# jie0530/act-plus-plus

Hardware: AMD Instinct MI355X
Metric: policy steps/sec (4x480x640 cams, chunk=100, bs=8) (higher is better)
Workload: dtype f32 (f16x3 split products: 3 fp16 MFMAs per fp32 product, fp32 accumulate); 1 GPU; ACT eval policy query: 4 cams 480x640 u8, chunk 100, hidden 512, ff 3200, 4 enc + 7 dec layers (layer 0 live), per-GPU batch 8, + temporal ensemble; per_gpu_batch=8, global_batch=8, parallelism=replicas x1

## Files before the change

act-plus-plus_amd/csrc/attn.hip:

```cpp
#include "common.h"
#include "dropout.h"
#include "split16.h"
#include <cstdio>
#include <cstdlib>

namespace {

constexpr bool ATTN_NOPF = true;
constexpr int KT = 64;
typedef _Float16 h16x8 __attribute__((ext_vector_type(8)));

__device__ __forceinline__ void attn_block_coords(int& bx, int& by, int& bz) {
    const int gx = gridDim.x, gy = gridDim.y;
    const int total = gx * gy * (int)gridDim.z;
    const int lin = ((int)blockIdx.z * gy + (int)blockIdx.y) * gx + (int)blockIdx.x;
    const int xcd = lin & 7, q = total >> 3, r = total & 7;
    const int base = (xcd < r) ? xcd * (q + 1) : r * (q + 1) + (xcd - r) * q;
    const int flat = base + (lin >> 3);
    bx = flat % gx;
    const int rest = flat / gx;
    by = rest % gy;
    bz = rest / gy;
}

template <int HD>
__global__ __launch_bounds__(256) void attn_f32_kernel(AttnArgs p, int nsplit, int chunk) {
    constexpr int HH = HD / 2;
    constexpr int DT = (HD + 31) / 32;
    constexpr int VD = DT * 32;
    constexpr int KS = HD + 4;
    __shared__ __attribute__((aligned(16))) float s_k[KT * KS];
    __shared__ __attribute__((aligned(16))) float s_v[KT * VD];

    const int t = threadIdx.x, lane = t & 63, wave = t >> 6;
    const int li = lane & 31, lh = lane >> 5;
    int bx, h, b;
    attn_block_coords(bx, h, b);
    const int split = bx % nsplit;
    const int q = (bx / nsplit) * 128 + wave * 32 + li;
    const int k_begin = split * chunk;
    const int k_end = (k_begin + chunk < p.Nk) ? k_begin + chunk : p.Nk;
    const bool qok = q < p.Nq;

    const float qscale = p.scale * 1.4426950408889634f;
    const float* Qp = p.Q + (int64_t)b * p.q_bs + (int64_t)(qok ? q : 0) * p.q_rs + h * HD + lh * HH;
    float qreg[HH];
#pragma unroll
    for (int s = 0; s < HH; s += 4) {
        f32x4 v = *reinterpret_cast<const f32x4*>(Qp + s);
#pragma unroll
        for (int j = 0; j < 4; ++j) qreg[s + j] = qok ? v[j] * qscale : 0.f;
    }
    const float* Kb = p.K + (int64_t)b * p.k_bs + h * HD;
    const float* Vb = p.V + (int64_t)b * p.v_bs + h * HD;
    const uint8_t* kpm = p.kpm ? p.kpm + (int64_t)b * p.kpm_bs : nullptr;

    f32x16 O[DT];
#pragma unroll
    for (int d = 0; d < DT; ++d)
#pragma unroll
        for (int e = 0; e < 16; ++e) O[d][e] = 0.f;
// ... 100 lines not shown
                for (int e = 0; e < 16; ++e) {
                    const int kl = sub * 32 + (e & 3) + 8 * (e >> 2) + 4 * lh;
#pragma unroll
                    for (int d = 0; d < DT; ++d) {
                        const float vv = s_v[kl * VD + d * 32 + li];
                        O[d] = __builtin_amdgcn_mfma_f32_32x32x2f32(vv, S[e], O[d], 0, 0, 0);
                    }
                }
            }
        }
        __syncthreads();
    }
    if (qok) {
        if (nsplit == 1) {
            const float inv = 1.f / l_run;
            float* Op = p.O + (int64_t)b * p.o_bs + (int64_t)q * p.o_rs + h * HD;
#pragma unroll
            for (int d = 0; d < DT; ++d)
#pragma unroll
                for (int g = 0; g < 4; ++g) {
                    const int d0 = d * 32 + 8 * g + 4 * lh;
                    if (d0 < HD) {
                        f32x4 o = {O[d][4 * g] * inv, O[d][4 * g + 1] * inv, O[d][4 * g + 2] * inv, O[d][4 * g + 3] * inv};
                        *reinterpret_cast<f32x4*>(Op + d0) = o;
                    }
                }
            if (p.lse && lh == 0) p.lse[((int64_t)b * p.H + h) * p.Nq + q] = m_run * 0.6931471805599453f + logf(l_run);
        } else {
            const int64_t row = (((int64_t)split * p.B + b) * p.H + h) * p.Nq + q;
            float* Op = p.ws + row * HD;
            float* ml = p.ws + (int64_t)nsplit * p.B * p.H * p.Nq * HD + row * 2;
#pragma unroll
            for (int d = 0; d < DT; ++d)
#pragma unroll
                for (int g = 0; g < 4; ++g) {
                    const int d0 = d * 32 + 8 * g + 4 * lh;
                    if (d0 < HD) {
                        f32x4 o = {O[d][4 * g], O[d][4 * g + 1], O[d][4 * g + 2], O[d][4 * g + 3]};
                        *reinterpret_cast<f32x4*>(Op + d0) = o;
                    }
                }
            if (lh == 0) { ml[0] = m_run; ml[1] = l_run; }
        }
    }
}

template <int HD>
__global__ __launch_bounds__(256, 3) void attn_f16x3_kernel(AttnArgs p, int nsplit, int chunk) {
    constexpr int NS = HD / 16;
    constexpr int DT = (HD + 31) / 32;
    constexpr int VD = DT * 32;
    constexpr int KROW = 4 * HD + 16;
    constexpr int VROW = 4 * KT + 16;
    __shared__ __attribute__((aligned(16))) unsigned char s_k[KT * KROW];
    __shared__ __attribute__((aligned(16))) unsigned char s_vt[VD * VROW];
    __shared__ uint8_t s_dead[KT];

    const int t = threadIdx.x, lane = t & 63, wave = t >> 6;
    const int li = lane & 31, lh = lane >> 5;
    int bx, h, b;
    attn_block_coords(bx, h, b);
    const int split = bx % nsplit;
    const int q = (bx / nsplit) * 128 + wave * 32 + li;
    const int k_begin = split * chunk;
    const int k_end = (k_begin + chunk < p.Nk) ? k_begin + chunk : p.Nk;
    const bool qok = q < p.Nq;

    const float qscale = p.scale * 1.4426950408889634f;
    const float* Qp = p.Q + (int64_t)b * p.q_bs + (int64_t)(qok ? q : 0) * p.q_rs + h * HD + lh * 8;
    h16x8 qh[NS], ql[NS];
#pragma unroll
    for (int s = 0; s < NS; ++s) {
        f32x4 v0 = *reinterpret_cast<const f32x4*>(Qp + s * 16);
        f32x4 v1 = *reinterpret_cast<const f32x4*>(Qp + s * 16 + 4);
        const float sc = qok ? qscale : 0.f;
        v0 *= sc; v1 *= sc;
        uint2 h0, l0, h1, l1;
        split16(v0, h0, l0);
        split16(v1, h1, l1);
        qh[s] = __builtin_bit_cast(h16x8, uint4{h0.x, h0.y, h1.x, h1.y});
        ql[s] = __builtin_bit_cast(h16x8, uint4{l0.x, l0.y, l1.x, l1.y});
    }
    const float* Kb = p.K + (int64_t)b * p.k_bs + h * HD;
    const float* Vb = p.V + (int64_t)b * p.v_bs + h * HD;
    const uint8_t* kpm = p.kpm ? p.kpm + (int64_t)b * p.kpm_bs : nullptr;

    f32x16 O[DT];
#pragma unroll
    for (int d = 0; d < DT; ++d)
#pragma unroll
        for (int e = 0; e < 16; ++e) O[d][e] = 0.f;
    float m_run = -INFINITY, l_run = 0.f;

    if (HD < VD) {
        for (int e = t; e < VD * VROW / 4; e += 256) reinterpret_cast<uint32_t*>(s_vt)[e] = 0u;
        __syncthreads();
    }

    constexpr int C4 = HD / 4;
    constexpr int NLK = (KT * C4 + 255) / 256;
    constexpr int NLV = (KT / 2 * C4 + 255) / 256;
    f32x4 pk[NLK], pv[NLV][2];
    auto vc = [&](int e) { return ((e >> 5) % (C4 / 4)) * 4 + (e & 3); };
    auto vkp = [&](int e) { return ((e >> 5) / (C4 / 4)) * 8 + ((e >> 2) & 7); };
    auto fetch = [&](int kt0) {
        const f32x4 z = {0.f, 0.f, 0.f, 0.f};
#pragma unroll
        for (int i = 0; i < NLK; ++i) {
            const int e = t + 256 * i;
            const int kr = e / C4, c = e - kr * C4;
            const int key = kt0 + kr;
            const bool ok = e < KT * C4 && key < k_end;
            const f32x4 kv = *reinterpret_cast<const f32x4*>(Kb + (ok ? (int64_t)key * p.k_rs + c * 4 : 0));
            pk[i] = ok ? kv : z;
        }
#pragma unroll
        for (int i = 0; i < NLV; ++i) {
            const int e = t + 256 * i;
            const int kp = vkp(e), c = vc(e);
#pragma unroll
            for (int u = 0; u < 2; ++u) {
                const int key = kt0 + 2 * kp + u;
                const bool ok = e < KT / 2 * C4 && key < k_end;
                const f32x4 vv = *reinterpret_cast<const f32x4*>(Vb + (ok ? (int64_t)key * p.v_rs + c * 4 : 0));
                pv[i][u] = ok ? vv : z;
            }
        }
    };
    if (!ATTN_NOPF) fetch(k_begin);
    for (int kt0 = k_begin; kt0 < k_end; kt0 += KT) {
        if (ATTN_NOPF) fetch(kt0);
#pragma unroll
        for (int i = 0; i < NLK; ++i) {
            const int e = t + 256 * i;
            if (e < KT * C4) {
                const int kr = e / C4, c = e - kr * C4;
                uint2 hi, lo;
                split16(pk[i], hi, lo);
                *reinterpret_cast<uint2*>(s_k + kr * KROW + c * 8) = hi;
                *reinterpret_cast<uint2*>(s_k + kr * KROW + 2 * HD + c * 8) = lo;
            }
        }
#pragma unroll
        for (int i = 0; i < NLV; ++i) {
            const int e = t + 256 * i;
            if (e < KT / 2 * C4) {
                const int kp = vkp(e), c = vc(e);
                uint2 ha, la, hb, lb;
                split16(pv[i][0], ha, la);
                split16(pv[i][1], hb, lb);
                const int kl = 2 * kp, r = kl & 15;
                const int pos = (kl & ~15) | (r & 3) | ((r & 8) >> 1) | ((r & 4) << 1);
                unsigned char* dst = s_vt + (c * 4) * VROW + pos * 2;
                *reinterpret_cast<uint32_t*>(dst + 0 * VROW) = (ha.x & 0xffffu) | (hb.x << 16);
                *reinterpret_cast<uint32_t*>(dst + 1 * VROW) = (ha.x >> 16) | (hb.x & 0xffff0000u);
                *reinterpret_cast<uint32_t*>(dst + 2 * VROW) = (ha.y & 0xffffu) | (hb.y << 16);
                *reinterpret_cast<uint32_t*>(dst + 3 * VROW) = (ha.y >> 16) | (hb.y & 0xffff0000u);
                *reinterpret_cast<uint32_t*>(dst + 0 * VROW + 2 * KT) = (la.x & 0xffffu) | (lb.x << 16);
                *reinterpret_cast<uint32_t*>(dst + 1 * VROW + 2 * KT) = (la.x >> 16) | (lb.x & 0xffff0000u);
                *reinterpret_cast<uint32_t*>(dst + 2 * VROW + 2 * KT) = (la.y & 0xffffu) | (lb.y << 16);
                *reinterpret_cast<uint32_t*>(dst + 3 * VROW + 2 * KT) = (la.y >> 16) | (lb.y & 0xffff0000u);
            }
        }
        const bool ragged = kt0 + KT > k_end || kpm != nullptr;
        if (ragged && t < KT) {
            const int key = kt0 + t;
            s_dead[t] = (key >= k_end) || (kpm && kpm[key] != 0);
        }
        __syncthreads();
        if (!ATTN_NOPF && kt0 + KT < k_end) fetch(kt0 + KT);
#pragma unroll
        for (int sub = 0; sub < KT / 32; ++sub) {
            const int kb = kt0 + sub * 32;
            if (kb < k_end) {
                f32x16 S;
#pragma unroll
                for (int e = 0; e < 16; ++e) S[e] = 0.f;
                const unsigned char* krow = s_k + (sub * 32 + li) * KROW + lh * 16;
#pragma unroll
                for (int s = 0; s < NS; ++s) {
                    const h16x8 kh = __builtin_bit_cast(h16x8, *reinterpret_cast<const f32x4*>(krow + s * 32));
                    const h16x8 kl = __builtin_bit_cast(h16x8, *reinterpret_cast<const f32x4*>(krow + 2 * HD + s * 32));
                    S = __builtin_amdgcn_mfma_f32_32x32x16_f16(kl, qh[s], S, 0, 0, 0);
                    S = __builtin_amdgcn_mfma_f32_32x32x16_f16(kh, ql[s], S, 0, 0, 0);
                    S = __builtin_amdgcn_mfma_f32_32x32x16_f16(kh, qh[s], S, 0, 0, 0);
                }
                if (ragged) {
#pragma unroll
                    for (int e = 0; e < 16; ++e)
                        if (s_dead[sub * 32 + (e & 3) + 8 * (e >> 2) + 4 * lh]) S[e] = -INFINITY;
                }
                if (p.causal) {
#pragma unroll
                    for (int e = 0; e < 16; ++e)
                        if (kb + (e & 3) + 8 * (e >> 2) + 4 * lh > q) S[e] = -INFINITY;
                }
                float mt = S[0];
#pragma unroll
                for (int e = 1; e < 16; ++e) mt = fmaxf(mt, S[e]);
                mt = fmaxf(mt, __shfl_xor(mt, 32, 64));
                const float m_new = fmaxf(m_run, mt);
                const float m_safe = (m_new == -INFINITY) ? 0.f : m_new;
                const float alpha = __builtin_amdgcn_exp2f(m_run - m_safe);
                float rs = 0.f;
#pragma unroll
                for (int e = 0; e < 16; ++e) {
                    S[e] = __builtin_amdgcn_exp2f(S[e] - m_safe);
                    rs += S[e];
                }
                rs += __shfl_xor(rs, 32, 64);
                l_run = l_run * alpha + rs;
                m_run = m_new;
                if (p.drop_p > 0.f) {
                    const float ds = 1.f / (1.f - p.drop_p);
                    const uint64_t rowbase = (((uint64_t)b * p.H + h) * p.Nq + (qok ? q : 0)) * (uint64_t)p.Nk;
#pragma unroll
                    for (int e = 0; e < 16; ++e) {
                        const int key = kb + (e & 3) + 8 * (e >> 2) + 4 * lh;
                        S[e] = actmi_keep(p.drop_seed, rowbase + key, p.drop_p) ? S[e] * ds : 0.f;
                    }
                }
                h16x8 ph[2], pl[2];
#pragma unroll
                for (int g2 = 0; g2 < 2; ++g2) {
                    const f32x4 a0 = {S[8 * g2], S[8 * g2 + 1], S[8 * g2 + 2], S[8 * g2 + 3]};
                    const f32x4 a1 = {S[8 * g2 + 4], S[8 * g2 + 5], S[8 * g2 + 6], S[8 * g2 + 7]};
                    uint2 h0, l0, h1, l1;
                    split16(a0, h0, l0);
                    split16(a1, h1, l1);
                    ph[g2] = __builtin_bit_cast(h16x8, uint4{h0.x, h0.y, h1.x, h1.y});
                    pl[g2] = __builtin_bit_cast(h16x8, uint4{l0.x, l0.y, l1.x, l1.y});
                }
#pragma unroll
                for (int d = 0; d < DT; ++d) {
#pragma unroll
                    for (int e = 0; e < 16; ++e) O[d][e] *= alpha;
                    const unsigned char* vrow = s_vt + (d * 32 + li) * VROW + sub * 64 + lh * 16;
#pragma unroll
                    for (int g2 = 0; g2 < 2; ++g2) {
                        const h16x8 vh = __builtin_bit_cast(h16x8, *reinterpret_cast<const f32x4*>(vrow + g2 * 32));
                        const h16x8 vl = __builtin_bit_cast(h16x8, *reinterpret_cast<const f32x4*>(vrow + 2 * KT + g2 * 32));
                        O[d] = __builtin_amdgcn_mfma_f32_32x32x16_f16(vl, ph[g2], O[d], 0, 0, 0);
                        O[d] = __builtin_amdgcn_mfma_f32_32x32x16_f16(vh, pl[g2], O[d], 0, 0, 0);
                        O[d] = __builtin_amdgcn_mfma_f32_32x32x16_f16(vh, ph[g2], O[d], 0, 0, 0);
                    }
                }
            }
        }
        __syncthreads();
    }
    if (qok) {
        if (nsplit == 1) {
            const float inv = 1.f / l_run;
            float* Op = p.O + (int64_t)b * p.o_bs + (int64_t)q * p.o_rs + h * HD;
#pragma unroll
            for (int d = 0; d < DT; ++d)
#pragma unroll
                for (int g = 0; g < 4; ++g) {
                    const int d0 = d * 32 + 8 * g + 4 * lh;
                    if (d0 < HD) {
                        f32x4 o = {O[d][4 * g] * inv, O[d][4 * g + 1] * inv, O[d][4 * g + 2] * inv, O[d][4 * g + 3] * inv};
                        *reinterpret_cast<f32x4*>(Op + d0) = o;
                    }
                }
            if (p.lse && lh == 0) p.lse[((int64_t)b * p.H + h) * p.Nq + q] = m_run * 0.6931471805599453f + logf(l_run);
        } else {
            const int64_t row = (((int64_t)split * p.B + b) * p.H + h) * p.Nq + q;
            float* Op = p.ws + row * HD;
            float* ml = p.ws + (int64_t)nsplit * p.B * p.H * p.Nq * HD + row * 2;
#pragma unroll
            for (int d = 0; d < DT; ++d)
#pragma unroll
                for (int g = 0; g < 4; ++g) {
                    const int d0 = d * 32 + 8 * g + 4 * lh;
                    if (d0 < HD) {
                        f32x4 o = {O[d][4 * g], O[d][4 * g + 1], O[d][4 * g + 2], O[d][4 * g + 3]};
                        *reinterpret_cast<f32x4*>(Op + d0) = o;
                    }
                }
            if (lh == 0) { ml[0] = m_run; ml[1] = l_run; }
        }
    }
}


__global__ void attn_combine_kernel(AttnArgs p, int nsplit, int HD) {
    const int64_t idx = (int64_t)blockIdx.x * blockDim.x + threadIdx.x;
    const int D4 = HD / 4;
    const int64_t total = (int64_t)p.B * p.H * p.Nq * D4;
    if (idx >= total) return;
    const int d4 = (int)(idx % D4);
    const int64_t bhq = idx / D4;
    const int q = (int)(bhq % p.Nq);
    const int h = (int)((bhq / p.Nq) % p.H);
    const int b = (int)(bhq / ((int64_t)p.Nq * p.H));
    const int64_t per = (int64_t)p.B * p.H * p.Nq;
    const float* mlb = p.ws + (int64_t)nsplit * per * HD;
    float m = -INFINITY;
    for (int s = 0; s < nsplit; ++s) m = fmaxf(m, mlb[(s * per + bhq) * 2]);
// ... 73 lines not shown
```

act-plus-plus_amd/csrc/conv3.hip:

```cpp
#include "common.h"
#include "split16.h"

namespace {

typedef _Float16 h16x8 __attribute__((ext_vector_type(8)));

constexpr int TR = 4, TW = 32, CH = 64;
constexpr int NTHR = TR * 64;
constexpr int PR = TR + 2, PW = TW + 2;
constexpr int PIX = 272;
constexpr int PATCH = PR * PW * PIX;
constexpr int WROW = 272;
constexpr int WBUF = CH * WROW;
constexpr int SMEM = PATCH + WBUF;

__global__ __launch_bounds__(NTHR) void conv3x3_c64_f16x3_kernel(Conv3Args p, int tiles_w, int tiles_h) {
    extern __shared__ __attribute__((aligned(16))) unsigned char smem[];
    unsigned char* s_patch = smem;
    unsigned char* s_w = smem + PATCH;
    const int t = threadIdx.x, lane = t & 63, wave = t >> 6;
    const int li = lane & 31, lh = lane >> 5;

    int tile;
    {
        const int total = (int)gridDim.x, lin = (int)blockIdx.x;
        const int xcd = lin & 7, q = total >> 3, r = total & 7;
        const int base = (xcd < r) ? xcd * (q + 1) : r * (q + 1) + (xcd - r) * q;
        tile = base + (lin >> 3);
    }
    const int tw = tile % tiles_w; tile /= tiles_w;
    const int th = tile % tiles_h; tile /= tiles_h;
    const int64_t img = tile;
    const int g = (int)(img / p.B);
    const int h0 = th * TR, w0 = tw * TW;
    const float* xin = p.x + img * (int64_t)p.H * p.W * CH;
    const float* wsplit = p.w16 + (int64_t)g * CH * 9 * CH;

    constexpr int WD = 4;
    constexpr int NWG = 1024 / NTHR;
    uint4 wreg[WD][NWG];
    auto fetch_w = [&](int tap, uint4 (&wr)[NWG]) {
#pragma unroll
        for (int i = 0; i < NWG; ++i) {
            const int e = t + NTHR * i;
            const int n = e >> 4, grp = e & 15;
            wr[i] = *reinterpret_cast<const uint4*>(wsplit + ((int64_t)n * 9 + tap) * CH + grp * 4);
        }
    };
    auto commit_w = [&](int buf, const uint4 (&wr)[NWG]) {
        unsigned char* dst = s_w;
#pragma unroll
        for (int i = 0; i < NWG; ++i) {
            const int e = t + NTHR * i;
            const int n = e >> 4, grp = e & 15;
            *reinterpret_cast<uint2*>(dst + n * WROW + grp * 8) = uint2{wr[i].x, wr[i].y};
            *reinterpret_cast<uint2*>(dst + n * WROW + 128 + grp * 8) = uint2{wr[i].z, wr[i].w};
        }
    };
#pragma unroll
    for (int k = 0; k < WD; ++k) fetch_w(k, wreg[k]);

    constexpr int NP = (PR * PW * 16 + NTHR - 1) / NTHR;
    const float xs = p.x_scale_dev ? *p.x_scale_dev : 1.f;
    const unsigned amax_seen = p.amax_out ? __hip_atomic_load(p.amax_out, __ATOMIC_RELAXED, __HIP_MEMORY_SCOPE_AGENT) : 0u;
    f32x4 pv[NP];
#pragma unroll
    for (int i = 0; i < NP; ++i) {
        const int e = t + NTHR * i;
        const int grp = e & 15, pix = e >> 4;
        const int pr = pix / PW, pc = pix - pr * PW;
        const int hi = h0 - 1 + pr, wi = w0 - 1 + pc;
        const bool ok = e < PR * PW * 16 && (unsigned)hi < (unsigned)p.H && (unsigned)wi < (unsigned)p.W;
        const f32x4 v = *reinterpret_cast<const f32x4*>(xin + (ok ? ((int64_t)hi * p.W + wi) * CH + grp * 4 : 0));
        pv[i] = ok ? v : f32x4{0.f, 0.f, 0.f, 0.f};
    }
#pragma unroll
    for (int i = 0; i < NP; ++i) {
        const int e = t + NTHR * i;
        if (e < PR * PW * 16) {
            const int grp = e & 15, pix = e >> 4;
            uint2 hv, lv;
            split16(pv[i] * xs, hv, lv);
            *reinterpret_cast<uint2*>(s_patch + pix * PIX + grp * 8) = hv;
            *reinterpret_cast<uint2*>(s_patch + pix * PIX + 128 + grp * 8) = lv;
        }
    }
    commit_w(0, wreg[0]);
    __syncthreads();

    f32x16 acc[2];
#pragma unroll
    for (int nt = 0; nt < 2; ++nt)
#pragma unroll
        for (int e = 0; e < 16; ++e) acc[nt][e] = 0.f;

#pragma unroll
    for (int tap = 0; tap < 9; ++tap) {
        const int buf = 0;
        if (tap + WD < 9) fetch_w(tap + WD, wreg[tap % WD]);
        const int r = tap / 3, s = tap - r * 3;
        const unsigned char* ap = s_patch + ((wave + r) * PW + li + s) * PIX + lh * 16;
        const unsigned char* bp = s_w + li * WROW + lh * 16;
        uint4 fa[4][2], fb[4][2][2];
#pragma unroll
        for (int ks = 0; ks < 4; ++ks) {
            fa[ks][0] = *reinterpret_cast<const uint4*>(ap + ks * 32);
            fa[ks][1] = *reinterpret_cast<const uint4*>(ap + 128 + ks * 32);
#pragma unroll
            for (int nt = 0; nt < 2; ++nt) {
                fb[ks][nt][0] = *reinterpret_cast<const uint4*>(bp + nt * 32 * WROW + ks * 32);
                fb[ks][nt][1] = *reinterpret_cast<const uint4*>(bp + nt * 32 * WROW + 128 + ks * 32);
            }
        }
#pragma unroll
        for (int ks = 0; ks < 4; ++ks) {
            const h16x8 xh = __builtin_bit_cast(h16x8, fa[ks][0]), xl = __builtin_bit_cast(h16x8, fa[ks][1]);
#pragma unroll
            for (int nt = 0; nt < 2; ++nt) {
                const h16x8 yh = __builtin_bit_cast(h16x8, fb[ks][nt][0]), yl = __builtin_bit_cast(h16x8, fb[ks][nt][1]);
                acc[nt] = __builtin_amdgcn_mfma_f32_32x32x16_f16(xl, yh, acc[nt], 0, 0, 0);
                acc[nt] = __builtin_amdgcn_mfma_f32_32x32x16_f16(xh, yl, acc[nt], 0, 0, 0);
                acc[nt] = __builtin_amdgcn_mfma_f32_32x32x16_f16(xh, yh, acc[nt], 0, 0, 0);
            }
        }
        __syncthreads();
        if (tap + 1 < 9) { commit_w(buf, wreg[(tap + 1) % WD]); __syncthreads(); }
    }

    const int ho = h0 + wave;
    constexpr int RS = CH + 4;
    float* scr = reinterpret_cast<float*>(s_patch) + wave * (TW * RS);
#pragma unroll
    for (int nt = 0; nt < 2; ++nt)
#pragma unroll
        for (int e = 0; e < 16; ++e)
            scr[((e & 3) + 8 * (e >> 2) + 4 * lh) * RS + nt * 32 + li] = acc[nt][e];
    if (ho >= p.H) return;
    const int c4 = lane & 15, pq = lane >> 4;
    const float inv = 1.f / (p.w_scale * xs);
    const f32x4 one4 = {1.f, 1.f, 1.f, 1.f}, zero4 = {0.f, 0.f, 0.f, 0.f};
    const f32x4 sc4 = (p.scale ? *reinterpret_cast<const f32x4*>(p.scale + g * CH + c4 * 4) : one4) * inv;
    const f32x4 bi4 = p.bias ? *reinterpret_cast<const f32x4*>(p.bias + g * CH + c4 * 4) : zero4;
    const f32x4 ps4 = p.post_scale ? *reinterpret_cast<const f32x4*>(p.post_scale + g * CH + c4 * 4) : one4;
    unsigned amx = 0;
    const int64_t rowbase = ((img * p.H + ho) * (int64_t)p.W) * CH + c4 * 4;
    f32x4 rv[8];
    if (p.res) {
#pragma unroll
        for (int q = 0; q < 8; ++q) {
            const int wo = w0 + q * 4 + pq;
            rv[q] = *reinterpret_cast<const f32x4*>(p.res + rowbase + (int64_t)(wo < p.W ? wo : 0) * CH);
        }
    }
#pragma unroll
    for (int q = 0; q < 8; ++q) {
        const int px = q * 4 + pq, wo = w0 + px;
        f32x4 v = *reinterpret_cast<const f32x4*>(scr + px * RS + c4 * 4) * sc4 + bi4;
        if (p.res) v += rv[q];
        if (p.relu) {
#pragma unroll
            for (int e = 0; e < 4; ++e) v[e] = fmaxf(v[e], 0.f);
        }
        if (wo < p.W) {
            if (p.mask) {
                const f32x4 mk = *reinterpret_cast<const f32x4*>(p.mask + rowbase + (int64_t)wo * CH);
#pragma unroll
                for (int e = 0; e < 4; ++e) v[e] = mk[e] > 0.f ? v[e] : 0.f;
            }
            v = v * ps4;
            *reinterpret_cast<f32x4*>(p.out + rowbase + (int64_t)wo * CH) = v;
#pragma unroll
            for (int e = 0; e < 4; ++e) amx = max(amx, __float_as_uint(v[e]) & 0x7fffffffu);
        }
    }
    if (p.amax_out) {
        for (int o = 32; o > 0; o >>= 1) amx = max(amx, (unsigned)__shfl_xor((int)amx, o, 64));
        if (lane == 0 && amx > amax_seen) atomicMax(p.amax_out, amx);
    }
}

}

int launch_conv3x3_c64(const Conv3Args& a, hipStream_t st, std::string* err) {
    if (a.H <= 0 || a.W <= 0 || a.B <= 0 || a.G <= 0) return 0;
    if (((uintptr_t)a.x & 15) || ((uintptr_t)a.w16 & 15)) { if (err) *err = "conv3x3_c64: pointers must be 16-byte aligned"; return -2; }
    if (!(a.w_scale > 0.f)) { if (err) *err = "conv3x3_c64: w_scale must be the (positive) scale of the split weight image"; return -2; }
    const int tiles_w = (a.W + TW - 1) / TW, tiles_h = (a.H + TR - 1) / TR;
    const int64_t blocks = (int64_t)a.G * a.B * tiles_h * tiles_w;
    static bool attr_set = false;
    if (!attr_set) {
        if (hipFuncSetAttribute(reinterpret_cast<const void*>(conv3x3_c64_f16x3_kernel), hipFuncAttributeMaxDynamicSharedMemorySize, SMEM) != hipSuccess) {
            if (err) *err = "conv3x3_c64: cannot raise the dynamic LDS limit";
            return -3;
        }
        attr_set = true;
    }
    const double px = (double)a.G * a.B * a.H * a.W;
    prof_begin("conv3x3_c64_f16x3_kernel", 2.0 * px * CH * 9 * CH, 4.0 * (px * CH * (a.res ? 3.0 : 2.0) + (double)a.G * CH * 9 * CH), st);
    hipLaunchKernelGGL(conv3x3_c64_f16x3_kernel, dim3((unsigned)blocks), dim3(NTHR), SMEM, st, a, tiles_w, tiles_h);
    prof_end(st);
    hipError_t e = hipGetLastError();
    if (e != hipSuccess) { if (err) *err = std::string("conv3x3_c64 launch: ") + hipGetErrorString(e); return -3; }
    return 0;
}
```

Baseline: 1735 policy steps/s.

## Software-pipeline f16x3 attention with double-buffered K, buffer loads and fast path

Adds a fast path for full tiles without mask, causal or dropout. K tiles are double-buffered in shared memory and the next tile's K and current V global loads are issued during the QK/softmax and PV MFMA work. Loads use raw buffer descriptors with precomputed offsets in place of predicated pointer loads, and a generic edge loop handles ragged tails. Shared memory for K doubles, which may reduce occupancy at the 3-blocks launch bound and raises register pressure from in-flight prefetch.

```diff
diff --git a/act-plus-plus_amd/csrc/attn.hip b/act-plus-plus_amd/csrc/attn.hip
--- a/act-plus-plus_amd/csrc/attn.hip
+++ b/act-plus-plus_amd/csrc/attn.hip
@@ -3,10 +3,10 @@
 #include "split16.h"
 #include <cstdio>
 #include <cstdlib>
+#include <type_traits>
 
 namespace {
 
-constexpr bool ATTN_NOPF = true;
 constexpr int KT = 64;
 typedef _Float16 h16x8 __attribute__((ext_vector_type(8)));
 
@@ -213,7 +213,7 @@
     constexpr int VD = DT * 32;
     constexpr int KROW = 4 * HD + 16;
     constexpr int VROW = 4 * KT + 16;
-    __shared__ __attribute__((aligned(16))) unsigned char s_k[KT * KROW];
+    __shared__ __attribute__((aligned(16))) unsigned char s_k[2 * KT * KROW];
     __shared__ __attribute__((aligned(16))) unsigned char s_vt[VD * VROW];
     __shared__ uint8_t s_dead[KT];
 
@@ -261,10 +261,12 @@
     constexpr int C4 = HD / 4;
     constexpr int NLK = (KT * C4 + 255) / 256;
     constexpr int NLV = (KT / 2 * C4 + 255) / 256;
+    static_assert(KT * C4 % 256 == 0, "every thread owns NLK K items");
+    constexpr bool VALL = KT / 2 * C4 % 256 == 0;
     f32x4 pk[NLK], pv[NLV][2];
     auto vc = [&](int e) { return ((e >> 5) % (C4 / 4)) * 4 + (e & 3); };
     auto vkp = [&](int e) { return ((e >> 5) / (C4 / 4)) * 8 + ((e >> 2) & 7); };
-    auto fetch = [&](int kt0) {
+    auto fetch_edge = [&](int kt0) {
         const f32x4 z = {0.f, 0.f, 0.f, 0.f};
 #pragma unroll
         for (int i = 0; i < NLK; ++i) {
@@ -288,24 +290,45 @@
             }
         }
     };
-    if (!ATTN_NOPF) fetch(k_begin);
-    for (int kt0 = k_begin; kt0 < k_end; kt0 += KT) {
-        if (ATTN_NOPF) fetch(kt0);
+    const unsigned k_offb = ((unsigned)(t / C4) * (unsigned)p.k_rs + (unsigned)(t % C4) * 4u) * 4u;
+    const unsigned v_offb = ((unsigned)(2 * vkp(t)) * (unsigned)p.v_rs + (unsigned)vc(t) * 4u) * 4u;
+    const int64_t k_rowb = p.k_rs * 4, v_rowb = p.v_rs * 4;
+    auto rsrc = [&](const float* base, int64_t rowb) {
+        return __builtin_amdgcn_make_buffer_rsrc(const_cast<float*>(base), 0, (int)((p.Nk - 1) * rowb + HD * 4), 0x00020000);
+    };
+    const __amdgpu_buffer_rsrc_t k_rsrc = rsrc(Kb, k_rowb), v_rsrc = rsrc(Vb, v_rowb);
+    auto ldb4 = [](__amdgpu_buffer_rsrc_t r, unsigned voffb, unsigned soffb) {
+        return __builtin_bit_cast(f32x4, __builtin_amdgcn_raw_buffer_load_b128(r, (int)voffb, (int)soffb, 0));
+    };
+    auto fetch_k = [&](int kt0) {
+#pragma unroll
+        for (int i = 0; i < NLK; ++i) pk[i] = ldb4(k_rsrc, k_offb, (unsigned)(kt0 + i * (256 / C4)) * (unsigned)k_rowb);
+    };
+    auto fetch_v = [&](int kt0) {
+        if (VALL || t < KT / 2 * C4) {
+#pragma unroll
+            for (int i = 0; i < NLV; ++i)
+#pragma unroll
+                for (int u = 0; u < 2; ++u)
+                    pv[i][u] = ldb4(v_rsrc, v_offb, (unsigned)(kt0 + i * (128 / (C4 / 4)) + u) * (unsigned)v_rowb);
+        }
+    };
+    auto stage_k = [&](unsigned char* sk) {
 #pragma unroll
         for (int i = 0; i < NLK; ++i) {
             const int e = t + 256 * i;
-            if (e < KT * C4) {
-                const int kr = e / C4, c = e - kr * C4;
-                uint2 hi, lo;
-                split16(pk[i], hi, lo);
-                *reinterpret_cast<uint2*>(s_k + kr * KROW + c * 8) = hi;
-                *reinterpret_cast<uint2*>(s_k + kr * KROW + 2 * HD + c * 8) = lo;
-            }
-        }
+            const int kr = e / C4, c = e - kr * C4;
+            uint2 hi, lo;
+            split16(pk[i], hi, lo);
+            *reinterpret_cast<uint2*>(sk + kr * KROW + c * 8) = hi;
+            *reinterpret_cast<uint2*>(sk + kr * KROW + 2 * HD + c * 8) = lo;
+        }
+    };
+    auto stage_v = [&]() {
 #pragma unroll
         for (int i = 0; i < NLV; ++i) {
             const int e = t + 256 * i;
-            if (e < KT / 2 * C4) {
+            if (VALL || e < KT / 2 * C4) {
                 const int kp = vkp(e), c = vc(e);
                 uint2 ha, la, hb, lb;
                 split16(pv[i][0], ha, la);
@@ -323,89 +346,132 @@
                 *reinterpret_cast<uint32_t*>(dst + 3 * VROW + 2 * KT) = (la.y >> 16) | (lb.y & 0xffff0000u);
             }
         }
+    };
+    auto qk_softmax = [&](auto edgec, const unsigned char* sk, int kt0, int sub, bool ragged, h16x8 (&ph)[2], h16x8 (&pl)[2],
+                          float& alpha) {
+        constexpr bool EDGE = decltype(edgec)::value;
+        const int kb = kt0 + sub * 32;
+        f32x16 S;
+#pragma unroll
+        for (int e = 0; e < 16; ++e) S[e] = 0.f;
+        const unsigned char* krow = sk + (sub * 32 + li) * KROW + lh * 16;
+#pragma unroll
+        for (int s = 0; s < NS; ++s) {
+            const h16x8 kh = __builtin_bit_cast(h16x8, *reinterpret_cast<const f32x4*>(krow + s * 32));
+            const h16x8 kl = __builtin_bit_cast(h16x8, *reinterpret_cast<const f32x4*>(krow + 2 * HD + s * 32));
+            S = __builtin_amdgcn_mfma_f32_32x32x16_f16(kl, qh[s], S, 0, 0, 0);
+            S = __builtin_amdgcn_mfma_f32_32x32x16_f16(kh, ql[s], S, 0, 0, 0);
+            S = __builtin_amdgcn_mfma_f32_32x32x16_f16(kh, qh[s], S, 0, 0, 0);
+        }
+        if (EDGE && ragged) {
+#pragma unroll
+            for (int e = 0; e < 16; ++e)
+                if (s_dead[sub * 32 + (e & 3) + 8 * (e >> 2) + 4 * lh]) S[e] = -INFINITY;
+        }
+        if (EDGE && p.causal) {
+#pragma unroll
+            for (int e = 0; e < 16; ++e)
+                if (kb + (e & 3) + 8 * (e >> 2) + 4 * lh > q) S[e] = -INFINITY;
+        }
+        float mt = S[0];
+#pragma unroll
+        for (int e = 1; e < 16; ++e) mt = fmaxf(mt, S[e]);
+        mt = fmaxf(mt, __shfl_xor(mt, 32, 64));
+        const float m_new = fmaxf(m_run, mt);
+        const float m_safe = (m_new == -INFINITY) ? 0.f : m_new;
+        alpha = __builtin_amdgcn_exp2f(m_run - m_safe);
+        float rs = 0.f;
+#pragma unroll
+        for (int e = 0; e < 16; ++e) {
+            S[e] = __builtin_amdgcn_exp2f(S[e] - m_safe);
+            rs += S[e];
+        }
+        rs += __shfl_xor(rs, 32, 64);
+        l_run = l_run * alpha + rs;
+        m_run = m_new;
+        if (EDGE && p.drop_p > 0.f) {
+            const float ds = 1.f / (1.f - p.drop_p);
+            const uint64_t rowbase = (((uint64_t)b * p.H + h) * p.Nq + (qok ? q : 0)) * (uint64_t)p.Nk;
+#pragma unroll
+            for (int e = 0; e < 16; ++e) {
+                const int key = kb + (e & 3) + 8 * (e >> 2) + 4 * lh;
+                S[e] = actmi_keep(p.drop_seed, rowbase + key, p.drop_p) ? S[e] * ds : 0.f;
+            }
+        }
+#pragma unroll
+        for (int g2 = 0; g2 < 2; ++g2) {
+            const f32x4 a0 = {S[8 * g2], S[8 * g2 + 1], S[8 * g2 + 2], S[8 * g2 + 3]};
+            const f32x4 a1 = {S[8 * g2 + 4], S[8 * g2 + 5], S[8 * g2 + 6], S[8 * g2 + 7]};
+            uint2 h0, l0, h1, l1;
+            split16(a0, h0, l0);
+            split16(a1, h1, l1);
+            ph[g2] = __builtin_bit_cast(h16x8, uint4{h0.x, h0.y, h1.x, h1.y});
+            pl[g2] = __builtin_bit_cast(h16x8, uint4{l0.x, l0.y, l1.x, l1.y});
+        }
+    };
+    auto pv_accum = [&](int sub, const h16x8 (&ph)[2], const h16x8 (&pl)[2], float alpha) {
+#pragma unroll
+        for (int d = 0; d < DT; ++d) {
+#pragma unroll
+            for (int e = 0; e < 16; ++e) O[d][e] *= alpha;
+            const unsigned char* vrow = s_vt + (d * 32 + li) * VROW + sub * 64 + lh * 16;
+#pragma unroll
+            for (int g2 = 0; g2 < 2; ++g2) {
+                const h16x8 vh = __builtin_bit_cast(h16x8, *reinterpret_cast<const f32x4*>(vrow + g2 * 32));
+                const h16x8 vl = __builtin_bit_cast(h16x8, *reinterpret_cast<const f32x4*>(vrow + 2 * KT + g2 * 32));
+                O[d] = __builtin_amdgcn_mfma_f32_32x32x16_f16(vl, ph[g2], O[d], 0, 0, 0);
+                O[d] = __builtin_amdgcn_mfma_f32_32x32x16_f16(vh, pl[g2], O[d], 0, 0, 0);
+                O[d] = __builtin_amdgcn_mfma_f32_32x32x16_f16(vh, ph[g2], O[d], 0, 0, 0);
+            }
+        }
+    };
+
+    int kt0 = k_begin;
+    const bool fast = kpm == nullptr && !p.causal && !(p.drop_p > 0.f) &&
+                      (int64_t)p.Nk * (p.k_rs > p.v_rs ? p.k_rs : p.v_rs) * 4 < (int64_t)1 << 31;
+    if (fast && kt0 + KT <= k_end) {
+        int cur = 0;
+        fetch_k(kt0);
+        stage_k(s_k);
+        for (;;) {
+            h16x8 ph[2], pl[2];
+            float alpha;
+            __syncthreads();
+            fetch_v(kt0);
+            qk_softmax(std::false_type{}, s_k + cur * (KT * KROW), kt0, 0, false, ph, pl, alpha);
+            __builtin_amdgcn_sched_barrier(0);
+            stage_v();
+            __syncthreads();
+            const bool more = kt0 + 2 * KT <= k_end;
+            if (more) fetch_k(kt0 + KT);
+            pv_accum(0, ph, pl, alpha);
+            qk_softmax(std::false_type{}, s_k + cur * (KT * KROW), kt0, 1, false, ph, pl, alpha);
+            pv_accum(1, ph, pl, alpha);
+            kt0 += KT;
+            if (!more) break;
+            cur ^= 1;
+            __builtin_amdgcn_sched_barrier(0);
+            stage_k(s_k + cur * (KT * KROW));
+        }
+        __syncthreads();
+    }
+    for (; kt0 < k_end; kt0 += KT) {
+        fetch_edge(kt0);
+        stage_k(s_k);
+        stage_v();
         const bool ragged = kt0 + KT > k_end || kpm != nullptr;
         if (ragged && t < KT) {
             const int key = kt0 + t;
             s_dead[t] = (key >= k_end) || (kpm && kpm[key] != 0);
         }
         __syncthreads();
-        if (!ATTN_NOPF && kt0 + KT < k_end) fetch(kt0 + KT);
 #pragma unroll
         for (int sub = 0; sub < KT / 32; ++sub) {
-            const int kb = kt0 + sub * 32;
-            if (kb < k_end) {
-                f32x16 S;
-#pragma unroll
-                for (int e = 0; e < 16; ++e) S[e] = 0.f;
-                const unsigned char* krow = s_k + (sub * 32 + li) * KROW + lh * 16;
-#pragma unroll
-                for (int s = 0; s < NS; ++s) {
-                    const h16x8 kh = __builtin_bit_cast(h16x8, *reinterpret_cast<const f32x4*>(krow + s * 32));
-                    const h16x8 kl = __builtin_bit_cast(h16x8, *reinterpret_cast<const f32x4*>(krow + 2 * HD + s * 32));
-                    S = __builtin_amdgcn_mfma_f32_32x32x16_f16(kl, qh[s], S, 0, 0, 0);
-                    S = __builtin_amdgcn_mfma_f32_32x32x16_f16(kh, ql[s], S, 0, 0, 0);
-                    S = __builtin_amdgcn_mfma_f32_32x32x16_f16(kh, qh[s], S, 0, 0, 0);
-                }
-                if (ragged) {
-#pragma unroll
-                    for (int e = 0; e < 16; ++e)
-                        if (s_dead[sub * 32 + (e & 3) + 8 * (e >> 2) + 4 * lh]) S[e] = -INFINITY;
-                }
-                if (p.causal) {
-#pragma unroll
-                    for (int e = 0; e < 16; ++e)
-                        if (kb + (e & 3) + 8 * (e >> 2) + 4 * lh > q) S[e] = -INFINITY;
-                }
-                float mt = S[0];
-#pragma unroll
-                for (int e = 1; e < 16; ++e) mt = fmaxf(mt, S[e]);
-                mt = fmaxf(mt, __shfl_xor(mt, 32, 64));
-                const float m_new = fmaxf(m_run, mt);
-                const float m_safe = (m_new == -INFINITY) ? 0.f : m_new;
-                const float alpha = __builtin_amdgcn_exp2f(m_run - m_safe);
-                float rs = 0.f;
-#pragma unroll
-                for (int e = 0; e < 16; ++e) {
-                    S[e] = __builtin_amdgcn_exp2f(S[e] - m_safe);
-                    rs += S[e];
-                }
-                rs += __shfl_xor(rs, 32, 64);
-                l_run = l_run * alpha + rs;
-                m_run = m_new;
-                if (p.drop_p > 0.f) {
-                    const float ds = 1.f / (1.f - p.drop_p);
-                    const uint64_t rowbase = (((uint64_t)b * p.H + h) * p.Nq + (qok ? q : 0)) * (uint64_t)p.Nk;
-#pragma unroll
-                    for (int e = 0; e < 16; ++e) {
-                        const int key = kb + (e & 3) + 8 * (e >> 2) + 4 * lh;
-                        S[e] = actmi_keep(p.drop_seed, rowbase + key, p.drop_p) ? S[e] * ds : 0.f;
-                    }
-                }
+            if (kt0 + sub * 32 < k_end) {
                 h16x8 ph[2], pl[2];
-#pragma unroll
-                for (int g2 = 0; g2 < 2; ++g2) {
-                    const f32x4 a0 = {S[8 * g2], S[8 * g2 + 1], S[8 * g2 + 2], S[8 * g2 + 3]};
-                    const f32x4 a1 = {S[8 * g2 + 4], S[8 * g2 + 5], S[8 * g2 + 6], S[8 * g2 + 7]};
-                    uint2 h0, l0, h1, l1;
-                    split16(a0, h0, l0);
-                    split16(a1, h1, l1);
-                    ph[g2] = __builtin_bit_cast(h16x8, uint4{h0.x, h0.y, h1.x, h1.y});
-                    pl[g2] = __builtin_bit_cast(h16x8, uint4{l0.x, l0.y, l1.x, l1.y});
-                }
-#pragma unroll
-                for (int d = 0; d < DT; ++d) {
-#pragma unroll
-                    for (int e = 0; e < 16; ++e) O[d][e] *= alpha;
-                    const unsigned char* vrow = s_vt + (d * 32 + li) * VROW + sub * 64 + lh * 16;
-#pragma unroll
-                    for (int g2 = 0; g2 < 2; ++g2) {
-                        const h16x8 vh = __builtin_bit_cast(h16x8, *reinterpret_cast<const f32x4*>(vrow + g2 * 32));
-                        const h16x8 vl = __builtin_bit_cast(h16x8, *reinterpret_cast<const f32x4*>(vrow + 2 * KT + g2 * 32));
-                        O[d] = __builtin_amdgcn_mfma_f32_32x32x16_f16(vl, ph[g2], O[d], 0, 0, 0);
-                        O[d] = __builtin_amdgcn_mfma_f32_32x32x16_f16(vh, pl[g2], O[d], 0, 0, 0);
-                        O[d] = __builtin_amdgcn_mfma_f32_32x32x16_f16(vh, ph[g2], O[d], 0, 0, 0);
-                    }
-                }
+                float alpha;
+                qk_softmax(std::true_type{}, s_k, kt0, sub, ragged, ph, pl, alpha);
+                pv_accum(sub, ph, pl, alpha);
             }
         }
         __syncthreads();
```

After: 1739 policy steps/s, median of 6. No clear change (+0.2%).

## Make conv3x3 blocks persistent over vertical strips with rolling halo patch

Applied to the files above, without the earlier changes.

Each block now walks a segment of consecutive row tiles down a column strip. It keeps a ring of patch rows in LDS and loads only the four new input rows per step, so the 2-row halo is not reloaded. Weight staging switches to half-tap granularity with a 6-deep register ring that carries over across steps, and launch bounds ask for two blocks per CU. The segment length is picked on the host from the CU count to balance wave quantization against per-block startup cost. In exchange, weights are re-streamed for every tile step and there is a barrier per half-tap, which adds sync overhead and register pressure.

```diff
diff --git a/act-plus-plus_amd/csrc/conv3.hip b/act-plus-plus_amd/csrc/conv3.hip
--- a/act-plus-plus_amd/csrc/conv3.hip
+++ b/act-plus-plus_amd/csrc/conv3.hip
@@ -9,174 +9,254 @@
 constexpr int NTHR = TR * 64;
 constexpr int PR = TR + 2, PW = TW + 2;
 constexpr int PIX = 272;
-constexpr int PATCH = PR * PW * PIX;
+constexpr int PROW = PW * PIX;
+constexpr int PATCH = PR * PROW;
 constexpr int WROW = 272;
 constexpr int WBUF = CH * WROW;
 constexpr int SMEM = PATCH + WBUF;
-
-__global__ __launch_bounds__(NTHR) void conv3x3_c64_f16x3_kernel(Conv3Args p, int tiles_w, int tiles_h) {
+constexpr int RS = CH + 4;
+static_assert(TW * RS * 4 <= PROW, "a wave's epilogue scratch must fit into one patch row slot");
+
+__global__ __launch_bounds__(NTHR, 2) void conv3x3_c64_f16x3_kernel(Conv3Args p, int tiles_w, int tiles_h, int seg_len, int nseg) {
     extern __shared__ __attribute__((aligned(16))) unsigned char smem[];
     unsigned char* s_patch = smem;
     unsigned char* s_w = smem + PATCH;
     const int t = threadIdx.x, lane = t & 63, wave = t >> 6;
     const int li = lane & 31, lh = lane >> 5;
 
-    int tile;
+    int unit;
     {
         const int total = (int)gridDim.x, lin = (int)blockIdx.x;
         const int xcd = lin & 7, q = total >> 3, r = total & 7;
         const int base = (xcd < r) ? xcd * (q + 1) : r * (q + 1) + (xcd - r) * q;
-        tile = base + (lin >> 3);
-    }
-    const int tw = tile % tiles_w; tile /= tiles_w;
-    const int th = tile % tiles_h; tile /= tiles_h;
-    const int64_t img = tile;
+        unit = base + (lin >> 3);
+    }
+    const int tw = unit % tiles_w; unit /= tiles_w;
+    const int seg = unit % nseg; unit /= nseg;
+    const int64_t img = unit;
     const int g = (int)(img / p.B);
-    const int h0 = th * TR, w0 = tw * TW;
+    const int th0 = seg * seg_len;
+    const int nsteps = min(seg_len, tiles_h - th0);
+    const int w0 = tw * TW;
     const float* xin = p.x + img * (int64_t)p.H * p.W * CH;
     const float* wsplit = p.w16 + (int64_t)g * CH * 9 * CH;
 
-    constexpr int WD = 4;
-    constexpr int NWG = 1024 / NTHR;
+    constexpr int NH = 18, WD = 6;
+    constexpr int NWG = 512 / NTHR;
+    static_assert(NH % WD == 0, "register ring must line up with the tile step");
     uint4 wreg[WD][NWG];
-    auto fetch_w = [&](int tap, uint4 (&wr)[NWG]) {
+    auto fetch_w = [&](int h, uint4 (&wr)[NWG]) {
+        const int tap = h >> 1, half = h & 1;
 #pragma unroll
         for (int i = 0; i < NWG; ++i) {
             const int e = t + NTHR * i;
-            const int n = e >> 4, grp = e & 15;
+            const int n = e >> 3, grp = (e & 7) + 8 * half;
             wr[i] = *reinterpret_cast<const uint4*>(wsplit + ((int64_t)n * 9 + tap) * CH + grp * 4);
         }
     };
-    auto commit_w = [&](int buf, const uint4 (&wr)[NWG]) {
-        unsigned char* dst = s_w;
+    auto commit_w = [&](int h, const uint4 (&wr)[NWG]) {
+        const int half = h & 1;
 #pragma unroll
         for (int i = 0; i < NWG; ++i) {
             const int e = t + NTHR * i;
-            const int n = e >> 4, grp = e & 15;
-            *reinterpret_cast<uint2*>(dst + n * WROW + grp * 8) = uint2{wr[i].x, wr[i].y};
-            *reinterpret_cast<uint2*>(dst + n * WROW + 128 + grp * 8) = uint2{wr[i].z, wr[i].w};
+            const int n = e >> 3, grp = (e & 7) + 8 * half;
+            *reinterpret_cast<uint2*>(s_w + n * WROW + grp * 8) = uint2{wr[i].x, wr[i].y};
+            *reinterpret_cast<uint2*>(s_w + n * WROW + 128 + grp * 8) = uint2{wr[i].z, wr[i].w};
         }
     };
 #pragma unroll
     for (int k = 0; k < WD; ++k) fetch_w(k, wreg[k]);
 
-    constexpr int NP = (PR * PW * 16 + NTHR - 1) / NTHR;
     const float xs = p.x_scale_dev ? *p.x_scale_dev : 1.f;
     const unsigned amax_seen = p.amax_out ? __hip_atomic_load(p.amax_out, __ATOMIC_RELAXED, __HIP_MEMORY_SCOPE_AGENT) : 0u;
-    f32x4 pv[NP];
-#pragma unroll
-    for (int i = 0; i < NP; ++i) {
-        const int e = t + NTHR * i;
-        const int grp = e & 15, pix = e >> 4;
-        const int pr = pix / PW, pc = pix - pr * PW;
-        const int hi = h0 - 1 + pr, wi = w0 - 1 + pc;
-        const bool ok = e < PR * PW * 16 && (unsigned)hi < (unsigned)p.H && (unsigned)wi < (unsigned)p.W;
-        const f32x4 v = *reinterpret_cast<const f32x4*>(xin + (ok ? ((int64_t)hi * p.W + wi) * CH + grp * 4 : 0));
-        pv[i] = ok ? v : f32x4{0.f, 0.f, 0.f, 0.f};
-    }
-#pragma unroll
-    for (int i = 0; i < NP; ++i) {
-        const int e = t + NTHR * i;
-        if (e < PR * PW * 16) {
+
+    {
+        constexpr int NP = (PR * PW * 16 + NTHR - 1) / NTHR;
+        const int h0 = th0 * TR;
+        f32x4 pv[NP];
+#pragma unroll
+        for (int i = 0; i < NP; ++i) {
+            const int e = t + NTHR * i;
             const int grp = e & 15, pix = e >> 4;
-            uint2 hv, lv;
-            split16(pv[i] * xs, hv, lv);
-            *reinterpret_cast<uint2*>(s_patch + pix * PIX + grp * 8) = hv;
-            *reinterpret_cast<uint2*>(s_patch + pix * PIX + 128 + grp * 8) = lv;
+            const int pr = pix / PW, pc = pix - pr * PW;
+            const int hi = h0 - 1 + pr, wi = w0 - 1 + pc;
+            const bool ok = e < PR * PW * 16 && (unsigned)hi < (unsigned)p.H && (unsigned)wi < (unsigned)p.W;
+            const f32x4 v = *reinterpret_cast<const f32x4*>(xin + (ok ? ((int64_t)hi * p.W + wi) * CH + grp * 4 : 0));
+            pv[i] = ok ? v : f32x4{0.f, 0.f, 0.f, 0.f};
+        }
+#pragma unroll
+        for (int i = 0; i < NP; ++i) {
+            const int e = t + NTHR * i;
+            if (e < PR * PW * 16) {
+                const int grp = e & 15, pix = e >> 4;
+                uint2 hv, lv;
+                split16(pv[i] * xs, hv, lv);
+                *reinterpret_cast<uint2*>(s_patch + pix * PIX + grp * 8) = hv;
+                *reinterpret_cast<uint2*>(s_patch + pix * PIX + 128 + grp * 8) = lv;
+            }
         }
     }
     commit_w(0, wreg[0]);
+    fetch_w(WD, wreg[0]);
     __syncthreads();
 
-    f32x16 acc[2];
-#pragma unroll
-    for (int nt = 0; nt < 2; ++nt)
-#pragma unroll
-        for (int e = 0; e < 16; ++e) acc[nt][e] = 0.f;
-
-#pragma unroll
-    for (int tap = 0; tap < 9; ++tap) {
-        const int buf = 0;
-        if (tap + WD < 9) fetch_w(tap + WD, wreg[tap % WD]);
-        const int r = tap / 3, s = tap - r * 3;
-        const unsigned char* ap = s_patch + ((wave + r) * PW + li + s) * PIX + lh * 16;
-        const unsigned char* bp = s_w + li * WROW + lh * 16;
-        uint4 fa[4][2], fb[4][2][2];
-#pragma unroll
-        for (int ks = 0; ks < 4; ++ks) {
-            fa[ks][0] = *reinterpret_cast<const uint4*>(ap + ks * 32);
-            fa[ks][1] = *reinterpret_cast<const uint4*>(ap + 128 + ks * 32);
-#pragma unroll
-            for (int nt = 0; nt < 2; ++nt) {
-                fb[ks][nt][0] = *reinterpret_cast<const uint4*>(bp + nt * 32 * WROW + ks * 32);
-                fb[ks][nt][1] = *reinterpret_cast<const uint4*>(bp + nt * 32 * WROW + 128 + ks * 32);
-            }
-        }
-#pragma unroll
-        for (int ks = 0; ks < 4; ++ks) {
-            const h16x8 xh = __builtin_bit_cast(h16x8, fa[ks][0]), xl = __builtin_bit_cast(h16x8, fa[ks][1]);
-#pragma unroll
-            for (int nt = 0; nt < 2; ++nt) {
-                const h16x8 yh = __builtin_bit_cast(h16x8, fb[ks][nt][0]), yl = __builtin_bit_cast(h16x8, fb[ks][nt][1]);
-                acc[nt] = __builtin_amdgcn_mfma_f32_32x32x16_f16(xl, yh, acc[nt], 0, 0, 0);
-                acc[nt] = __builtin_amdgcn_mfma_f32_32x32x16_f16(xh, yl, acc[nt], 0, 0, 0);
-                acc[nt] = __builtin_amdgcn_mfma_f32_32x32x16_f16(xh, yh, acc[nt], 0, 0, 0);
-            }
-        }
-        __syncthreads();
-        if (tap + 1 < 9) { commit_w(buf, wreg[(tap + 1) % WD]); __syncthreads(); }
-    }
-
-    const int ho = h0 + wave;
-    constexpr int RS = CH + 4;
-    float* scr = reinterpret_cast<float*>(s_patch) + wave * (TW * RS);
-#pragma unroll
-    for (int nt = 0; nt < 2; ++nt)
-#pragma unroll
-        for (int e = 0; e < 16; ++e)
-            scr[((e & 3) + 8 * (e >> 2) + 4 * lh) * RS + nt * 32 + li] = acc[nt][e];
-    if (ho >= p.H) return;
     const int c4 = lane & 15, pq = lane >> 4;
     const float inv = 1.f / (p.w_scale * xs);
     const f32x4 one4 = {1.f, 1.f, 1.f, 1.f}, zero4 = {0.f, 0.f, 0.f, 0.f};
-    const f32x4 sc4 = (p.scale ? *reinterpret_cast<const f32x4*>(p.scale + g * CH + c4 * 4) : one4) * inv;
-    const f32x4 bi4 = p.bias ? *reinterpret_cast<const f32x4*>(p.bias + g * CH + c4 * 4) : zero4;
-    const f32x4 ps4 = p.post_scale ? *reinterpret_cast<const f32x4*>(p.post_scale + g * CH + c4 * 4) : one4;
     unsigned amx = 0;
-    const int64_t rowbase = ((img * p.H + ho) * (int64_t)p.W) * CH + c4 * 4;
-    f32x4 rv[8];
-    if (p.res) {
-#pragma unroll
-        for (int q = 0; q < 8; ++q) {
-            const int wo = w0 + q * 4 + pq;
-            rv[q] = *reinterpret_cast<const f32x4*>(p.res + rowbase + (int64_t)(wo < p.W ? wo : 0) * CH);
-        }
-    }
-#pragma unroll
-    for (int q = 0; q < 8; ++q) {
-        const int px = q * 4 + pq, wo = w0 + px;
-        f32x4 v = *reinterpret_cast<const f32x4*>(scr + px * RS + c4 * 4) * sc4 + bi4;
-        if (p.res) v += rv[q];
-        if (p.relu) {
-#pragma unroll
-            for (int e = 0; e < 4; ++e) v[e] = fmaxf(v[e], 0.f);
-        }
-        if (wo < p.W) {
-            if (p.mask) {
-                const f32x4 mk = *reinterpret_cast<const f32x4*>(p.mask + rowbase + (int64_t)wo * CH);
-#pragma unroll
-                for (int e = 0; e < 4; ++e) v[e] = mk[e] > 0.f ? v[e] : 0.f;
-            }
-            v = v * ps4;
-            *reinterpret_cast<f32x4*>(p.out + rowbase + (int64_t)wo * CH) = v;
-#pragma unroll
-            for (int e = 0; e < 4; ++e) amx = max(amx, __float_as_uint(v[e]) & 0x7fffffffu);
+
+    constexpr int NR = (PW * 16 + 63) / 64;
+    f32x4 nv[NR];
+    const int ngrp = lane & 15, npc = lane >> 4;
+    const int64_t ncol = (int64_t)(w0 - 1 + npc) * CH + ngrp * 4;
+    unsigned nmask = 0;
+#pragma unroll
+    for (int i = 0; i < NR; ++i)
+        if (npc + 4 * i < PW && (unsigned)(w0 - 1 + npc + 4 * i) < (unsigned)p.W) nmask |= 1u << i;
+
+    int b = 0;
+#pragma nounroll
+    for (int step = 0; step < nsteps; ++step) {
+        const int h0 = (th0 + step) * TR;
+        const bool more = step + 1 < nsteps;
+        if (more) {
+            const int hi = h0 + TR + 1 + wave;
+            const unsigned m = hi < p.H ? nmask : 0u;
+            const int64_t roff = (int64_t)hi * p.W * CH + ncol;
+#pragma unroll
+            for (int i = 0; i < NR; ++i) {
+                nv[i] = zero4;
+                if (m >> i & 1) nv[i] = *reinterpret_cast<const f32x4*>(xin + roff + i * 4 * CH);
+            }
+        }
+
+        f32x16 acc[2];
+#pragma unroll
+        for (int nt = 0; nt < 2; ++nt)
+#pragma unroll
+            for (int e = 0; e < 16; ++e) acc[nt][e] = 0.f;
+
+        const unsigned char* bp = s_w + li * WROW + lh * 16;
+#pragma unroll
+        for (int h = 0; h < NH; ++h) {
+            const int tap = h >> 1, r = tap / 3, s = tap - r * 3;
+            int slot = b + wave + r; slot -= slot >= PR ? PR : 0;
+            const unsigned char* ap = s_patch + (slot * PW + li + s) * PIX + lh * 16;
+            uint4 fa[2][2], fb[2][2][2];
+#pragma unroll
+            for (int k = 0; k < 2; ++k) {
+                const int ks = 2 * (h & 1) + k;
+                fa[k][0] = *reinterpret_cast<const uint4*>(ap + ks * 32);
+                fa[k][1] = *reinterpret_cast<const uint4*>(ap + 128 + ks * 32);
+#pragma unroll
+                for (int nt = 0; nt < 2; ++nt) {
+                    fb[k][nt][0] = *reinterpret_cast<const uint4*>(bp + nt * 32 * WROW + ks * 32);
+                    fb[k][nt][1] = *reinterpret_cast<const uint4*>(bp + nt * 32 * WROW + 128 + ks * 32);
+                }
+            }
+            if (h + 1 < NH || more) commit_w((h + 1) % NH, wreg[(h + 1) % WD]);
+            if (h + 1 + WD < NH || more) fetch_w((h + 1 + WD) % NH, wreg[(h + 1) % WD]);
+#pragma unroll
+            for (int k = 0; k < 2; ++k) {
+                const h16x8 xh = __builtin_bit_cast(h16x8, fa[k][0]), xl = __builtin_bit_cast(h16x8, fa[k][1]);
+#pragma unroll
+                for (int nt = 0; nt < 2; ++nt) {
+                    const h16x8 yh = __builtin_bit_cast(h16x8, fb[k][nt][0]), yl = __builtin_bit_cast(h16x8, fb[k][nt][1]);
+                    acc[nt] = __builtin_amdgcn_mfma_f32_32x32x16_f16(xl, yh, acc[nt], 0, 0, 0);
+                    acc[nt] = __builtin_amdgcn_mfma_f32_32x32x16_f16(xh, yl, acc[nt], 0, 0, 0);
+                    acc[nt] = __builtin_amdgcn_mfma_f32_32x32x16_f16(xh, yh, acc[nt], 0, 0, 0);
+                }
+            }
+            __syncthreads();
+        }
+
+        const f32x4 sc4 = (p.scale ? *reinterpret_cast<const f32x4*>(p.scale + g * CH + c4 * 4) : one4) * inv;
+        const f32x4 bi4 = p.bias ? *reinterpret_cast<const f32x4*>(p.bias + g * CH + c4 * 4) : zero4;
+        const f32x4 ps4 = p.post_scale ? *reinterpret_cast<const f32x4*>(p.post_scale + g * CH + c4 * 4) : one4;
+        const int ho = h0 + wave;
+        int sslot = b + wave; sslot -= sslot >= PR ? PR : 0;
+        unsigned char* srow = s_patch + sslot * PROW;
+        float* scr = reinterpret_cast<float*>(srow);
+#pragma unroll
+        for (int nt = 0; nt < 2; ++nt)
+#pragma unroll
+            for (int e = 0; e < 16; ++e)
+                scr[((e & 3) + 8 * (e >> 2) + 4 * lh) * RS + nt * 32 + li] = acc[nt][e];
+        if (ho < p.H) {
+            const int64_t obase = ((img * p.H + ho) * (int64_t)p.W + w0 + pq) * CH + c4 * 4;
+            const int wleft = p.W - w0 - pq;
+            f32x4 rv[8];
+            if (p.res) {
+#pragma unroll
+                for (int q = 0; q < 8; ++q) {
+                    rv[q] = zero4;
+                    if (q * 4 < wleft) rv[q] = *reinterpret_cast<const f32x4*>(p.res + obase + q * 4 * CH);
+                }
+            }
+#pragma unroll
+            for (int q = 0; q < 8; ++q) {
+                const int px = q * 4 + pq;
+                f32x4 v = *reinterpret_cast<const f32x4*>(scr + px * RS + c4 * 4) * sc4 + bi4;
+                if (p.res) v += rv[q];
+                if (p.relu) {
+#pragma unroll
+                    for (int e = 0; e < 4; ++e) v[e] = fmaxf(v[e], 0.f);
+                }
+                if (q * 4 < wleft) {
+                    if (p.mask) {
+                        const f32x4 mk = *reinterpret_cast<const f32x4*>(p.mask + obase + q * 4 * CH);
+#pragma unroll
+                        for (int e = 0; e < 4; ++e) v[e] = mk[e] > 0.f ? v[e] : 0.f;
+                    }
+                    v = v * ps4;
+                    *reinterpret_cast<f32x4*>(p.out + obase + q * 4 * CH) = v;
+#pragma unroll
+                    for (int e = 0; e < 4; ++e) amx = max(amx, __float_as_uint(v[e]) & 0x7fffffffu);
+                }
+            }
+        }
+        if (more) {
+            asm volatile("" ::: "memory");
+#pragma unroll
+            for (int i = 0; i < NR; ++i) {
+                const int pc = npc + 4 * i;
+                if (pc < PW) {
+                    uint2 hv, lv;
+                    split16(nv[i] * xs, hv, lv);
+                    *reinterpret_cast<uint2*>(srow + pc * PIX + ngrp * 8) = hv;
+                    *reinterpret_cast<uint2*>(srow + pc * PIX + 128 + ngrp * 8) = lv;
+                }
+            }
+            b = b + TR >= PR ? b + TR - PR : b + TR;
+            __syncthreads();
         }
     }
     if (p.amax_out) {
         for (int o = 32; o > 0; o >>= 1) amx = max(amx, (unsigned)__shfl_xor((int)amx, o, 64));
         if (lane == 0 && amx > amax_seen) atomicMax(p.amax_out, amx);
     }
+}
+
+int cu_count() {
+    static int n = 0;
+    if (n <= 0) {
+        int dev = 0, v = 0;
+        if (hipGetDevice(&dev) == hipSuccess && hipDeviceGetAttribute(&v, hipDeviceAttributeMultiprocessorCount, dev) == hipSuccess && v > 0) n = v;
+        else return 256;
+    }
+    return n;
+}
+
+int pick_seg_len(int64_t strips, int tiles_h, int slots) {
+    constexpr double COLD = 0.5;
+    int best = 1;
+    double best_cost = 0.;
+    for (int len = 1; len <= tiles_h; ++len) {
+        const int ns = (tiles_h + len - 1) / len;
+        const double cost = (double)((strips * ns + slots - 1) / slots) * (len + COLD);
+        if (len == 1 || cost < best_cost) { best = len; best_cost = cost; }
+    }
+    return best;
 }
 
 }
@@ -186,7 +266,10 @@
     if (((uintptr_t)a.x & 15) || ((uintptr_t)a.w16 & 15)) { if (err) *err = "conv3x3_c64: pointers must be 16-byte aligned"; return -2; }
     if (!(a.w_scale > 0.f)) { if (err) *err = "conv3x3_c64: w_scale must be the (positive) scale of the split weight image"; return -2; }
     const int tiles_w = (a.W + TW - 1) / TW, tiles_h = (a.H + TR - 1) / TR;
-    const int64_t blocks = (int64_t)a.G * a.B * tiles_h * tiles_w;
+    const int64_t strips = (int64_t)a.G * a.B * tiles_w;
+    const int seg_len = pick_seg_len(strips, tiles_h, 2 * cu_count());
+    const int nseg = (tiles_h + seg_len - 1) / seg_len;
+    const int64_t blocks = strips * nseg;
     static bool attr_set = false;
     if (!attr_set) {
         if (hipFuncSetAttribute(reinterpret_cast<const void*>(conv3x3_c64_f16x3_kernel), hipFuncAttributeMaxDynamicSharedMemorySize, SMEM) != hipSuccess) {
@@ -197,7 +280,7 @@
     }
     const double px = (double)a.G * a.B * a.H * a.W;
     prof_begin("conv3x3_c64_f16x3_kernel", 2.0 * px * CH * 9 * CH, 4.0 * (px * CH * (a.res ? 3.0 : 2.0) + (double)a.G * CH * 9 * CH), st);
-    hipLaunchKernelGGL(conv3x3_c64_f16x3_kernel, dim3((unsigned)blocks), dim3(NTHR), SMEM, st, a, tiles_w, tiles_h);
+    hipLaunchKernelGGL(conv3x3_c64_f16x3_kernel, dim3((unsigned)blocks), dim3(NTHR), SMEM, st, a, tiles_w, tiles_h, seg_len, nseg);
     prof_end(st);
     hipError_t e = hipGetLastError();
     if (e != hipSuccess) { if (err) *err = std::string("conv3x3_c64 launch: ") + hipGetErrorString(e); return -3; }
```

Result: no change. 1764 policy steps/s before, 1768 policy steps/s after, median of 6 (+0.2%).
